# diaoenmao/Multimodal-Controller-for-Generative-Models

Measured on AMD Instinct MI355X. Metric: images/sec (train step) MCGAN CIFAR-10 32x32, higher is better.
Workload: dtype bf16

## Files before the change

multimodal-controller-for-generative-models_amd/csrc/conv_fused.hip:

```cpp
#include "conv_tile.h"
#include <stdlib.h>
#include <type_traits>

namespace {

template <typename T, int BM, int BN, int WM, int WN>
struct ConvCfg {
    static constexpr int NT = 64 * WM * WN;
    static constexpr int FM = BM / WM / 16;
    static constexpr int FN = BN / WN / 16;
    static constexpr int ESZ = Elem<T>::BYTES;
    static constexpr int APITCH = MCGEN_CK * ESZ + 16 * ESZ;
    static constexpr int BROW = MCGEN_CK * ESZ;
    static constexpr int BBYTES = BN * BROW;
    static constexpr int EP = BN + 4;
    static constexpr int NI = (BM * 9 + NT - 1) / NT;
    static constexpr int UPR = BROW / 16;
    static constexpr int UNITS = BN * UPR;
    static constexpr int NU = (UNITS + NT - 1) / NT;
    static constexpr int EPX = (BN >= 128 && BM > 64) ? BM / 64 : 1;
    static constexpr int PPX = BM / EPX;
    static constexpr int CH = BN / 8;
    static constexpr int PROWS = NT / CH;
    static_assert(NT % CH == 0, "epilogue thread mapping");
// ... 1611 lines not shown
    const int H = p.H, N = p.N;
    int tile_m = blockIdx.x;
    int wset = 0;
    if (p.order || p.wsel) {
        const int tpi = (H * W) / BM, pos = tile_m / tpi;
        if (p.wsel) wset = p.wsel[pos];
        if (p.order) tile_m = p.order[pos] * tpi + (tile_m - pos * tpi);
    }
    const int cout0 = blockIdx.y * BN;
    const Geo g = make_geo(BM, tile_m, H, W);
    const int n_img = g.n0 < N ? g.n0 : N - 1;

    f32x4 acc[FN][FM];
#pragma unroll
    for (int i = 0; i < FN; ++i)
#pragma unroll
        for (int j = 0; j < FM; ++j) acc[i][j] = f32x4{0.f, 0.f, 0.f, 0.f};

    const mcgen_seg_t sg0 = seg_for_tile(p.seg[0], g);
    const int C0 = sg0.C;
    const char* wimg = reinterpret_cast<const char*>(p.w) + (size_t)wset * (size_t)p.wsel_stride * 2;
    const size_t wblock_bytes = (size_t)p.Cout_w * BROW;
    auto seg_info = [&](int si, const int16_t*& cidx, int& cw, int& cnt) {
        const mcgen_seg_t& sg = p.seg[si];
        cw = sg.Cw > 0 ? sg.Cw : sg.C;
        cidx = nullptr; cnt = sg.C;
        if (sg.cmap) {
            const int16_t* rec = sg.cmap + (size_t)n_img * sg.cmap_stride;
            cidx = rec + cw;
            cnt = (int)mc_sload(rec + 2 * cw + 32 + 2 * ((cw + 31) >> 5));
            if (cnt > sg.C) cnt = sg.C;
        }
    };
    const int16_t* cidx0 = nullptr; int cw0 = C0, cnt0 = C0;
    if constexpr (GK) seg_info(0, cidx0, cw0, cnt0);
    const int nchunk = GK ? ((cnt0 + 31) >> 5) : (C0 >> 5), T0 = nchunk * 9;
    const size_t tapstride0 = (size_t)(cw0 + 1) * p.Cout_w * 2;

    constexpr int UPR = C::UPR, RPP = 64 / UPR;
    int d_src[PPW];
    int k0_[PPW];
    const int rsub = lane / LPR, ci = lane % LPR;
#pragma unroll
    for (int k = 0; k < PPW; ++k) {
        const int piece = wave * PPW + k;
        if constexpr (!GK) {
            const int row = piece * RPP + lane / UPR, pu = lane % UPR;
            const int lgrp = pu ^ (3 * ((row >> 3) & 1));
            d_src[k] = (cout0 + row < p.Cout_w) ? (cout0 + row) * BROW + lgrp * 16 : (lane % UPR) * 16;
            k0_[k] = 0;
        } else {
            const int rho0 = RPPK * piece, rho = rho0 + rsub;
            k0_[k] = (rho0 < 16) ? 8 * (rho0 >> 2) + (rho0 & 3) : 8 * ((rho0 - 16) >> 2) + 4 + ((rho0 - 16) & 3);
            int co = cout0 + 16 * ((ci >> 1) ^ (rho & 7)) + 8 * (ci & 1);
            if (co > p.Cout_w - 8) co = p.Cout_w - 8;
            d_src[k] = co * 2;
        }
    }
    auto ksel_map = [&](const int16_t* cidx, int t, int k) -> int {
        const uint32_t d01 = mc_sload(cidx + 32 * t + k0_[k]);
        uint32_t sel = d01;
        if constexpr (RPPK == 4) {
            const uint32_t d23 = mc_sload(cidx + 32 * t + k0_[k] + 2);
            sel = (rsub & 2) ? d23 : d01;
        }
        return (int)((rsub & 1) ? (sel >> 16) : (sel & 0xffffu));
    };
    auto ksel = [&](const int16_t* cidx, int cw, int t, int k) -> int {
        if (cidx) return ksel_map(cidx, t, k);
// ... 164 lines not shown
                    for (int i = 0; i < HF; ++i) M::run(wf[fn], af[cs][i], acc[fn][i]);
            } else {
                const int sn = (slot_c + 1 == R) ? 0 : slot_c + 1;
                const char* ldsB = ldsB0 + sn * BB;
#pragma unroll
                for (int fn = 0; fn < FN; ++fn) {
#pragma unroll
                    for (int i = 0; i < HF; ++i) M::run(wf[fn], af[cs][i], acc[fn][HF + i]);
                    wf[fn] = wfrag(ldsB, fn);
                }
            }
            if constexpr (h == 0) {
                asm volatile("s_waitcnt lgkmcnt(0)" ::: "memory");
                pp_wait_vm<pp_vmcnt_b(ph, R, NIW, PPW)>();
                pp_barrier();
            } else {
                slot_c = (slot_c + 1 == R) ? 0 : slot_c + 1;
                ++tcur;
            }
        });
        if constexpr (GK) {
#pragma unroll
            for (int kk = 0; kk < PPW; ++kk) krow_c[kk] = krow_n[kk];
        }
    }
    asm volatile("s_waitcnt vmcnt(0)" ::: "memory");
    }

    if (p.nseg > 1) {
        int tg = 0;
        int nrest = 0;
        const int16_t* cidx1 = nullptr; int cw1 = 8, cnt1 = 0;
        if constexpr (GK) { seg_info(1, cidx1, cw1, cnt1); nrest = (cnt1 + 31) >> 5; }
        else for (int s = 1; s < p.nseg; ++s) nrest += (p.seg[s].C + MCGEN_CK - 1) / MCGEN_CK;
        const char* wseg1 = wimg + 9 * tapstride0;
        const size_t tapstride1 = (size_t)(cw1 + 1) * p.Cout_w * 2;
        auto tail_dma = [&](int t, int slot) {
#pragma unroll
            for (int k = 0; k < PPW; ++k) {
                if constexpr (GK) dma_piece_gk(wseg1, tapstride1, ksel(cidx1, cw1, t, k) * p.Cout_w * 2 + d_src[k], 0, slot, k);
                else dma_piece(T0 + t, slot, k);
            }
        };
        pp_barrier();
        constexpr int SUBW = BM * APITCH;
        constexpr int A2 = 2 * (((PP * APITCH + 1023) / 1024) * 1024);
        constexpr int TGMAX = (A2 + 2 * BB) / SUBW;
#ifndef MCGEN_PP_TG
#define MCGEN_PP_TG 4
#endif
        constexpr int TG = TGMAX < MCGEN_PP_TG ? TGMAX : MCGEN_PP_TG;
        constexpr int NI1 = (BM * 4 + NT - 1) / NT;
        static_assert(TG >= 1 && R >= 5, "tail groups: windows over the window buffers + two ring slots, weights in slots 2 .. 4");
        auto tslot = [](int t) { return 2 + t % 3; };
        auto tail_dma_c = [&](int t) { tail_dma(t < nrest ? t : nrest - 1, tslot(t)); };
        if (nrest > 0) { tail_dma_c(0); tail_dma_c(1); }
        for (int s = 1; s < p.nseg; ++s) {
            const mcgen_seg_t sg = seg_for_tile(p.seg[s], g);
            PatchStager<T, NT, NI1, APITCH> stager;
            stager.setup(sg, g, N, H, W, tid);
            const int b_lane = (wm * (BM / WM) + l15) * APITCH + lg * 16;
            const int nch = GK ? nrest : (sg.C + MCGEN_CK - 1) / MCGEN_CK;
#pragma unroll 1
            for (int q0 = 0; q0 < nch; q0 += TG) {
                const int ng = (nch - q0) < TG ? (nch - q0) : TG;
                if (q0 > 0) __builtin_amdgcn_s_barrier();
                {
                    typename PatchStager<T, NT, NI1, APITCH>::raw_t raw[TG];
#pragma unroll
                    for (int i = 0; i < TG; ++i) if (i < ng) stager.load(sg, (q0 + i) * MCGEN_CK, raw[i]);
#pragma unroll
                    for (int i = 0; i < TG; ++i) if (i < ng) stager.write(sg, (q0 + i) * MCGEN_CK, raw[i], ldsA0 + i * SUBW, g.n0 < N ? g.n0 : -1);
                }
#pragma unroll 1
                for (int i = 0; i < ng; ++i) {
                    if constexpr (PPW == 2) asm volatile("s_waitcnt vmcnt(2)" ::: "memory"); else asm volatile("s_waitcnt vmcnt(1)" ::: "memory");
                    asm volatile("s_waitcnt lgkmcnt(0)" ::: "memory");
                    pp_barrier();
                    tail_dma_c(tg + 2);
                    const char* ldsB = ldsB0 + tslot(tg) * BB;
                    const char* ldsW = ldsA0 + i * SUBW + b_lane;
                    typename M::frag xf[FM], yf[FN];
#pragma unroll
                    for (int fm = 0; fm < FM; ++fm) xf[fm] = *reinterpret_cast<const typename M::frag*>(ldsW + fm * 16 * APITCH);
#pragma unroll
                    for (int fn = 0; fn < FN; ++fn) yf[fn] = wfrag(ldsB, fn);
#pragma unroll
                    for (int fn = 0; fn < FN; ++fn)
#pragma unroll
                        for (int fm = 0; fm < FM; ++fm) M::run(yf[fn], xf[fm], acc[fn][fm]);
                    ++tg;
                }
            }
        }
    }
// ... 256 lines not shown
    auto kern = conv_gk_kernel<BM, BN, WM, WN>;
    static int raised = 0;
    if (int rc = raise_lds(reinterpret_cast<const void*>(kern), lds, &raised)) return rc;
    hipLaunchKernelGGL(kern, dim3(mt, nt), dim3(C::NT), lds, st, *p, a_bytes);
    MCGEN_LAUNCH_CHECK("conv_fused(gk)");
    return 0;
}

static int dispatch_gk(const mcgen_conv_t* p, int dtype, hipStream_t st) {
    MCGEN_CHECK(dtype == MCGEN_BF16, "conv_fused: K-major launches are bf16");
    for (int s = 0; s < p->nseg; ++s) {
        const mcgen_seg_t& g = p->seg[s];
        const int cw = g.Cw > 0 ? g.Cw : g.C;
        MCGEN_CHECK(cw % 8 == 0 && cw <= 2048 && g.C <= cw + 32, "conv_fused(gk): segment %d: bad channel counts C=%d Cw=%d", s, g.C, cw);
        MCGEN_CHECK(g.cmap || g.C == cw, "conv_fused(gk): segment %d: compacted channels need the map that orders them", s);
        MCGEN_CHECK(!g.cmap || g.cmap_stride >= 2 * cw + 32, "conv_fused(gk): segment %d: map stride too small", s);
        MCGEN_CHECK(!g.cmap || g.code == nullptr, "conv_fused(gk): segment %d: the code of a compacted segment rides in its scale / shift rows", s);
    }
    MCGEN_CHECK(p->Cout_w % 8 == 0 && p->Cout_w >= 64, "conv_fused(gk): at least 64 output channels");
    int bm = 0, bn = 0;
    MCGEN_CHECK(mc_tile(p, &bm, &bn), "conv_fused(gk): no tile of a %dx%d map lies inside one image", p->H, p->W);
    static const long pp_mode = env_long("MCGEN_PP", 7);
    if (bm == 256 && bn == 256 && (pp_mode & 4) && pp_fits_<256, 256, 2, 4, 5, true>(p)) return launch_pp<bf16_t, 256, 256, 2, 4, 5, true>(p, st);
    if (bm == 256 && bn == 256) return launch_gk<256, 256, 2, 4>(p, st);
    if (bm == 128 && bn == 256) return launch_gk<128, 256, 2, 4>(p, st);
    return launch_gk<128, 128, 2, 2>(p, st);
}

template <int BM, int BN, int WM, int WN, int R, bool GK>
static bool pp_fits_(const mcgen_conv_t* p) {
    using C = ConvCfg<bf16_t, BM, BN, WM, WN>;
    if (p->w_layout != (GK ? 2 : 0) || p->H * p->W < BM || (p->W != 16 && p->W != 32)) return false;
    if (p->seg[0].ksize != 3 || p->seg[0].C % MCGEN_CK != 0 || p->seg[0].C < 2 * MCGEN_CK || p->seg[0].C > C::NT) return false;
    if ((p->seg[0].cmap != nullptr) != GK) return false;
    for (int s = 1; s < p->nseg; ++s) if (p->seg[s].ksize != 1 || (!GK && p->seg[s].cmap)) return false;
    const int PP = mcgen_patch_pixels(BM, p->H, p->W, 3);
    if (PP * 4 > PP_NIW_MAX * C::NT || PP * 4 <= C::NT) return false;
    const int a_bytes = round_up(PP * C::APITCH, 1024);
    const int lds = 2 * a_bytes + R * C::BBYTES + p->seg[0].C * 8 + 16;
    return lds <= 160 * 1024;
}
template <int BM, int BN, int WM, int WN, int R>
static bool pp_fits(const mcgen_conv_t* p) { return pp_fits_<BM, BN, WM, WN, R, false>(p); }
template <typename T, int BM, int BN, int WM, int WN, int R, bool GK>
static int launch_pp(const mcgen_conv_t* p, hipStream_t st) {
    static_assert(sizeof(T) == 2, "the pp form is bf16");
    using C = ConvCfg<bf16_t, BM, BN, WM, WN>;
    const long Mtot = (long)p->N * p->H * p->W;
    const int mt = (int)(Mtot / BM);
    const int nt = (p->Cout_w + BN - 1) / BN;
    const int PP = mcgen_patch_pixels(BM, p->H, p->W, 3);
    const int a_bytes = round_up(PP * C::APITCH, 1024);
    int lds = 2 * a_bytes + R * C::BBYTES + p->seg[0].C * 8 + 16;
    const int epi_bytes = C::PPX * C::EP * 4 + (p->ycmap ? YTAB_BYTES : 0), red_bytes = C::PROWS * BN * 2 * 4;
    const int epi_fast = (BM / PP_EPI_PASSES(BM, BN)) * C::EP * 4 + (p->ycmap ? YTAB_BYTES : 0);
    if (epi_bytes > lds) lds = epi_bytes;
    if (epi_fast > lds) lds = epi_fast;
    if (red_bytes > lds) lds = red_bytes;
    MCGEN_CHECK(lds <= 160 * 1024, "conv_fused(pp): tile %dx%d needs %d bytes of LDS", BM, BN, lds);
    void (*kern)(const mcgen_conv_t, const int) = p->W == 32 ? conv_pp_kernel<BM, BN, WM, WN, R, 5, GK> : conv_pp_kernel<BM, BN, WM, WN, R, 4, GK>;
#ifdef MCGEN_TUNING
    static const long abl = env_long("MCGEN_PP_ABL", 0);
    if (abl == 2 && p->W == 32) kern = conv_pp_kernel<BM, BN, WM, WN, R, 5, GK, 2>;
#endif
#ifdef MCGEN_TUNING
    int raised_now = 0;
    if (int rc = raise_lds(reinterpret_cast<const void*>(kern), lds, &raised_now)) return rc;
#else
// ... 41 lines not shown
#endif
    };
    *n = (int)(sizeof(t) / sizeof(t[0]));
    return t;
}

static int dispatch(const mcgen_conv_t* p, int dtype, const TilePick& t, hipStream_t st) {
    int n = 0;
    const CfgEntry* tab = dtype == MCGEN_BF16 ? bf16_table(&n) : f32_table(&n);
    for (int i = 0; i < n; ++i)
        if (tab[i].BM == t.BM && tab[i].BN == t.BN && tab[i].pipe == t.pipe) return tab[i].fn(p, st);
    return mcgen_fail("conv_fused: no instantiation for tile %dx%d pipe=%d dtype=%d", t.BM, t.BN, t.pipe, dtype);
}

static int validate(const mcgen_conv_t* p) {
    MCGEN_CHECK(p && p->nseg >= 1 && p->nseg <= 2, "conv_fused: nseg must be 1 or 2");
    MCGEN_CHECK(p->N > 0 && ilog2_exact(p->H) >= 0 && ilog2_exact(p->W) >= 0, "conv_fused: H and W must be powers of two (got %dx%d)", p->H, p->W);
    MCGEN_CHECK(p->W <= 64 && p->H * p->W >= 1, "conv_fused: W up to 64 supported");
    MCGEN_CHECK(p->Cout > 0 && p->Cout_w == round_up(p->Cout, 16), "conv_fused: Cout_w must be Cout rounded up to 16");
    MCGEN_CHECK(p->Cy % 8 == 0 && p->Cy > 0, "conv_fused: Cy must be a positive multiple of 8");
    MCGEN_CHECK(p->w && p->y, "conv_fused: null weight image or output");
    for (int s = 0; s < p->nseg; ++s) {
        const mcgen_seg_t& g = p->seg[s];
        MCGEN_CHECK(g.x && g.C > 0 && g.C % 8 == 0, "conv_fused: segment %d: C must be a positive multiple of 8", s);
        MCGEN_CHECK(g.ksize == 1 || g.ksize == 3, "conv_fused: segment %d: ksize must be 1 or 3", s);
        MCGEN_CHECK(!g.ups || (p->H >= 2 && p->W >= 2), "conv_fused: upsampled segment needs H, W >= 2");
        MCGEN_CHECK(g.group_n >= 0 && (g.group_n == 0 || p->N % g.group_n == 0), "conv_fused: segment %d: group_n must divide N", s);
    }
    if (p->pool) MCGEN_CHECK(p->H >= 2 && p->W >= 2, "conv_fused: pooling needs H, W >= 2");
    MCGEN_CHECK(p->stats_mode >= 0 && p->stats_mode <= 2, "conv_fused: bad stats_mode");
    MCGEN_CHECK(p->stats_mode != 2 || (p->gate_x && p->gmean && p->grstd), "conv_fused: stats_mode 2 needs gate_x, gmean, grstd");
    MCGEN_CHECK(p->stats_mode == 0 || p->stats, "conv_fused: stats_mode set without a stats buffer");
    MCGEN_CHECK(p->w_layout >= 0 && p->w_layout <= 2, "conv_fused: unknown weight layout %d", p->w_layout);
    if (p->wsel || p->order) {
        MCGEN_CHECK(p->w_layout == 0 && (p->y_group == 0 || !p->order), "conv_fused: per-mode weight sets (wsel / order) go with the chunked weight image (w_layout 0)");
        MCGEN_CHECK(!p->wsel || p->wsel_stride > 0, "conv_fused: wsel needs wsel_stride");
    }
    if (p->yperm) {
        MCGEN_CHECK(p->wsel && !p->order && !p->ycmap, "conv_fused: permuted weight rows (yperm) come with wsel, without order / ycmap");
        MCGEN_CHECK(!p->pool && !p->res && !p->gate_x && !p->ocode && !p->tanh_out, "conv_fused: a compacted output takes bias and statistics only");
        MCGEN_CHECK(p->Cy % 8 == 0 && p->Cy <= p->Cout && p->Cout % 8 == 0 && p->Cout_w == p->Cout && p->Cout_w <= 256 && p->yperm_stride >= p->Cout && p->yperm_stride % 8 == 0,
                    "conv_fused: yperm: bad pitch %d / stride %d for %d channels", p->Cy, p->yperm_stride, p->Cout);
    }
    if (p->ycmap) {
        MCGEN_CHECK(!p->pool && !p->res && !p->gate_x && !p->ocode && !p->tanh_out && !p->bias2, "conv_fused: a compacted output takes bias and statistics only");
        MCGEN_CHECK(p->Cy % 32 == 0 && p->Cy <= round_up(p->Cout, 8) + 32 && p->ycmap_stride >= 2 * round_up(p->Cout, 8) + 32,
                    "conv_fused: compacted output: bad pitch %d / map stride %d", p->Cy, p->ycmap_stride);
        MCGEN_CHECK(p->Cout_w <= 256, "conv_fused: a compacted output needs all channels in one tile");
    } else if (!p->yperm) {
        MCGEN_CHECK(p->Cy >= p->Cout, "conv_fused: Cy must be >= Cout");
    }
    return 0;
}

}

extern "C" int mcgen_conv_m_tiles(const mcgen_conv_t* p, int dtype) {
    if (!p) return 0;
    if (p->w_layout != 0) {
        int bm = 0, bn = 0;
        if (!mc_tile(p, &bm, &bn)) return 0;
        return (int)(((long)p->N * p->H * p->W + bm - 1) / bm);
    }
    if (mcgen_conv_smap_ok(p, dtype)) return p->N;
    if (const int bm = mcgen_conv_px1_bm(p, dtype)) return (int)((long)p->N * p->H * p->W / bm);
    const TilePick t = pick_tile(p, dtype);
// ... 2 lines not shown
}

extern "C" int mcgen_conv_tile(const mcgen_conv_t* p, int dtype, int* bm, int* bn) {
    if (!p || !bm || !bn) return mcgen_fail("conv_tile: null pointer");
    if (p->w_layout != 0) {
        MCGEN_CHECK(mc_tile(p, bm, bn), "conv_tile: no K-major tile for a %dx%d map", p->H, p->W);
        return 0;
    }
    const TilePick t = pick_tile(p, dtype);
    *bm = t.BM; *bn = t.BN;
    return 0;
}

extern "C" int mcgen_conv_form(const mcgen_conv_t* p, int dtype) {
    if (!p || p->w_layout != 0 || p->order) return 0;
    if (p->wsel) return mcgen_conv_head_ok(p, dtype) ? 5 : 0;
    if (mcgen_conv_skinny_ok(p, dtype)) return 1;
    if (mcgen_conv_smap_ok(p, dtype)) return 2;
    if (mcgen_conv_px1_bm(p, dtype)) return 3;
    if (mcgen_conv_c8_ok(p, dtype)) return 4;
    if (mcgen_conv_head_ok(p, dtype)) return 5;
    return 0;
}

extern "C" int mcgen_conv_fused(const mcgen_conv_t* p, int dtype, void* stream) {
    if (int rc = validate(p)) return rc;
    if (p->y_group != 0) {
        MCGEN_CHECK(mcgen_conv_head_ok(p, dtype), "conv_fused: the paired output layout (y_group) is built for the image head only "
                    "(bf16, one 3x3 segment to <= 8 channels of pitch 8 on 32x32 maps, N %% y_group == 0)");
        return mcgen_conv_head(p, reinterpret_cast<hipStream_t>(stream));
    }
    if (p->w_layout == 1) return dispatch_mc(p, dtype, reinterpret_cast<hipStream_t>(stream));
    if (p->w_layout == 2) return dispatch_gk(p, dtype, reinterpret_cast<hipStream_t>(stream));
    for (int s = 0; s < p->nseg; ++s) MCGEN_CHECK(p->seg[s].cmap == nullptr, "conv_fused: a compaction map needs a K-major launch (w_layout 1 or 2)");
    if (p->wsel && mcgen_conv_head_ok(p, dtype)) return mcgen_conv_head(p, reinterpret_cast<hipStream_t>(stream));
    if (p->wsel || p->order) {
        const TilePick tw = pick_tile(p, dtype);
        MCGEN_CHECK(dtype == MCGEN_BF16 && tw.pipe == 20, "conv_fused: per-mode weight sets need the software-pipelined bf16 form "
                    "(3x3 first segment of 64 .. 512 channels in whole chunks, 16x16 / 32x32 maps, >= 65536 pixels)");
        if (p->ycmap) MCGEN_CHECK(tw.BM <= p->H * p->W && p->Cout_w <= tw.BN, "conv_fused: compacted output: the %dx%d tile must hold all %d channels", tw.BM, tw.BN, p->Cout_w);
        if (p->yperm) MCGEN_CHECK(tw.BM <= p->H * p->W && p->Cout_w == tw.BN, "conv_fused: yperm: the %dx%d tile must hold exactly the %d channels", tw.BM, tw.BN, p->Cout_w);
        return dispatch(p, dtype, tw, reinterpret_cast<hipStream_t>(stream));
    }
    if (mcgen_conv_skinny_ok(p, dtype)) return mcgen_conv_skinny(p, reinterpret_cast<hipStream_t>(stream));
    if (mcgen_conv_smap_ok(p, dtype)) return mcgen_conv_smap(p, reinterpret_cast<hipStream_t>(stream));
    if (mcgen_conv_px1_bm(p, dtype)) return mcgen_conv_px1(p, reinterpret_cast<hipStream_t>(stream));
    if (mcgen_conv_c8_ok(p, dtype)) return mcgen_conv_c8(p, reinterpret_cast<hipStream_t>(stream));
    if (mcgen_conv_head_ok(p, dtype)) return mcgen_conv_head(p, reinterpret_cast<hipStream_t>(stream));
    const TilePick t = pick_tile(p, dtype);
    if (p->ycmap) MCGEN_CHECK(dtype == MCGEN_BF16 && t.BM <= p->H * p->W && p->Cout_w <= t.BN,
                              "conv_fused: compacted output: the %dx%d tile must lie inside one image and hold all %d channels", t.BM, t.BN, p->Cout_w);
    MCGEN_CHECK(t.BM >= 2 * p->W || p->H * p->W <= t.BM, "conv_fused: tile of %d pixels too small for W=%d", t.BM, p->W);
    for (int s = 0; s < p->nseg; ++s) {
        const int ti = t.BM > p->H * p->W ? t.BM / (p->H * p->W) : 1;
        MCGEN_CHECK(p->seg[s].group_n == 0 || p->seg[s].group_n % ti == 0,
                    "conv_fused: a tile of %d images would straddle BatchNorm groups of %d images", ti, p->seg[s].group_n);
    }
    hipStream_t st = reinterpret_cast<hipStream_t>(stream);
    if (dtype != MCGEN_F32 && dtype != MCGEN_BF16) return mcgen_fail("conv_fused: unknown dtype %d", dtype);
    return dispatch(p, dtype, t, st);
}
#endif
```

multimodal-controller-for-generative-models_amd/csrc/conv_head.hip:

```cpp
#include "conv_tile.h"

namespace {

constexpr int HD_NT = 512, HD_W = 32, HD_ROWS = 8;
constexpr int HD_PC = HD_W + 2, HD_PP = (HD_ROWS + 2) * HD_PC;
constexpr int HD_PITCH = 80;
constexpr int HD_BUF = ((HD_PP * HD_PITCH + 127) / 128) * 128;
constexpr int HD_NI = (HD_PP * 4 + HD_NT - 1) / HD_NT;

__global__ __launch_bounds__(HD_NT, 4)
void conv_head_kernel(const mcgen_conv_t p) {
    extern __shared__ __attribute__((aligned(16))) char smem[];
    const int tid = threadIdx.x, lane = tid & 63;
    const int wv = __builtin_amdgcn_readfirstlane(tid >> 6);
    const int l15 = lane & 15, lg = lane >> 4;
    const int n = blockIdx.x >> 2, h0 = (blockIdx.x & 3) * HD_ROWS;
    const mcgen_seg_t sg = p.seg[0];
    const int C = sg.C, nchunk = C >> 5;
    const float* anyf = reinterpret_cast<const float*>(p.w);
    const size_t arow = sg.group_n > 0 ? (size_t)(n / sg.group_n) * C : 0;
    const float* scp = sg.scale ? sg.scale + arow : anyf;
    const float* shp = sg.scale ? sg.shift + arow : anyf;
    const float* cdp = sg.code ? sg.code + (size_t)n * C : anyf;
    const float relu_lo = sg.relu ? 0.f : -__builtin_inff();

    const int u = tid & 3;
    int src[HD_NI], dst[HD_NI];
#pragma unroll
    for (int k = 0; k < HD_NI; ++k) {
        const int wp = (tid >> 2) + 128 * k;
        const int wr = wp / HD_PC, wc = wp - wr * HD_PC;
        const int h = h0 + wr - 1, w = wc - 1;
        dst[k] = wp < HD_PP ? wp * HD_PITCH + u * 16 : -1;
        src[k] = (wp < HD_PP && (unsigned)h < (unsigned)HD_W && (unsigned)w < (unsigned)HD_W) ? ((n * HD_W + h) * HD_W + w) * C + u * 8 : -1;
    }
    const bf16_t* xs = reinterpret_cast<const bf16_t*>(sg.x);
    u32x4 raw[HD_NI];
    float sc[8], sh[8], cd[8];
    auto load_chunk = [&](int q) {
#pragma unroll
        for (int k = 0; k < HD_NI; ++k) raw[k] = *reinterpret_cast<const u32x4*>(xs + (src[k] >= 0 ? (size_t)src[k] + q * 32 : 0));
        load8f(sg.scale ? scp + q * 32 + u * 8 : anyf, sc);
        load8f(sg.scale ? shp + q * 32 + u * 8 : anyf, sh);
        load8f(sg.code ? cdp + q * 32 + u * 8 : anyf, cd);
    };
    auto write_chunk = [&](char* buf) {
#pragma unroll
        for (int k = 0; k < HD_NI; ++k) {
            if (dst[k] < 0) continue;
            union { bf16x8 h; u32x4 w; } o;
#pragma unroll
// ... 29 lines not shown
            }
        }
        if (q + 1 < nchunk) write_chunk(smem + ((q + 1) & 1) * HD_BUF);
    }
    if (lg < 2) {
        float bs[4];
#pragma unroll
        for (int r = 0; r < 4; ++r) {
            const int co = 4 * lg + r;
            bs[r] = (p.bias && co < p.Cout) ? p.bias[co] : 0.f;
            if (p.bias2 && co < p.Cout) bs[r] += p.bias2[co];
        }
        const int ny = p.y_group > 0 ? (n / p.y_group) * 2 * p.y_group + p.y_group + n % p.y_group : n;
        bf16_t* y = reinterpret_cast<bf16_t*>(p.y) + ((size_t)(ny * HD_W + h0 + wv) * HD_W) * p.Cy + 4 * lg;
#pragma unroll
        for (int f = 0; f < 2; ++f) {
            union { bf16_t h[4]; uint2 w; } o;
#pragma unroll
            for (int r = 0; r < 4; ++r) {
                float v = fmaf(acc[f][r], p.alpha, bs[r]);
                if (p.tanh_out) v = tanhf(v);
                o.h[r] = (bf16_t)((4 * lg + r) < p.Cout ? v : 0.f);
            }
            *reinterpret_cast<uint2*>(y + (size_t)(16 * f + l15) * p.Cy) = o.w;
        }
    }
}

}

int mcgen_conv_head_ok(const mcgen_conv_t* p, int dtype) {
    if (dtype != MCGEN_BF16 || p->w_layout != 0 || p->nseg != 1) return 0;
    const mcgen_seg_t& g = p->seg[0];
    if (g.ksize != 3 || g.ups || g.cmap || g.C % 32 || g.C < 64 || g.group_n < 0 || (g.group_n > 0 && p->N % g.group_n)) return 0;
    if (p->H != HD_W || p->W != HD_W || p->Cout > 8 || p->Cout_w != 16 || p->Cy != 8) return 0;
    if (p->pool || p->res || p->ocode || p->gate_x || p->stats_mode || p->ycmap || p->order) return 0;
    if ((long)p->N * HD_W * HD_W * g.C >= (1L << 31)) return 0;
    if (p->y_group < 0 || (p->y_group > 0 && p->N % p->y_group)) return 0;
    return 1;
}

int mcgen_conv_head(const mcgen_conv_t* p, hipStream_t st) {
    static bool raised = false;
    if (!raised) {
        raised = true;
        hipError_t e = hipFuncSetAttribute(reinterpret_cast<const void*>(conv_head_kernel), hipFuncAttributeMaxDynamicSharedMemorySize, 2 * HD_BUF);
        if (e != hipSuccess) return mcgen_fail("conv_head: cannot raise LDS limit: %s", hipGetErrorString(e));
    }
    hipLaunchKernelGGL(conv_head_kernel, dim3(p->N * 4), dim3(HD_NT), 2 * HD_BUF, st, *p);
    MCGEN_LAUNCH_CHECK("conv_head");
    return 0;
}
```

multimodal-controller-for-generative-models_amd/gan_engine.py:

```python
from __future__ import annotations

from typing import Dict, List, Optional

import torch
import torch.nn as nn

from . import ops
from ._tuning import flag as _flag
from .ops import Seg

Tensor = torch.Tensor


def _bump(t: Tensor):
    torch.autograd.graph.increment_version(t)


class FlatState:

    def __init__(self, tensors: List[Tensor]):
        self.tensors = tensors
        self.flat: Optional[Tensor] = None
        self.offsets: List[int] = []
        self._index = {id(t): i for i, t in enumerate(tensors)}
# ... 378 lines not shown
        c0 = lin.out_features // 16
        x0, st = ops.conv_fused([Seg(zt, ksize=1)], self.img['lin'], 16 * c0, bias=self.img['lin_bias'],
                                stats_mode=st_mode)
        x = x0.view(n, 4, 4, c0)
        fold = 16
        ctx['zt'] = zt
        blocks_ctx = []
        codes = self._codes.run_any(indicator)
        gk = groups > 1 and one_hot and self._gk_enabled()
        hint = getattr(indicator, '_mcgen_onehot', None)
        pm = gk and self._pm_enabled() and hint is not None and hint[0].shape[0] * hint[1] == n
        wsel = None
        if pm:
            wsel = hint[2] if len(hint) > 2 and hint[2] is not None else hint[0].to(torch.int32).repeat(hint[1])
        x_cm = None
        cmaps = self._gather_cmaps(self._pm_need(), wsel) if pm else {}
        caps_h = [self._cap(b.mc_2) if (gk and self._gk_block(i)) else None for i, b in enumerate(res)]
        for i, b in enumerate(res):
            s = x.shape[1]
            code1, code2 = codes[2 * i], codes[2 * i + 1]
            bn1 = _bn_forward(b.conv[0].module, st, ng * s * s, train, fold, groups)
            fold = 1
            co = b.conv[4].module.out_channels
            ci = b.conv[4].module.in_channels
            cap_h = caps_h[i]
            nxt = res[i + 1] if i + 1 < len(res) else None
            ymc = self._y_mc(i, pm and 'headm' in self.img) if cap_h is not None else None
            cap_y = self._cap(ymc) if ymc is not None else None
            cm_h = (cmaps[id(b.mc_2)] if id(b.mc_2) in cmaps else ops.mc_cmap(code2)) if cap_h else None
            cm_y = (cmaps[id(ymc)] if id(ymc) in cmaps else ops.mc_cmap(codes[2 * (i + 1)])) if cap_y else None
            if x_cm is not None:
                sa, ta = ops.mc_affine(code1, x_cm[0], x_cm[1], bn1.scale, bn1.shift, group_n=gn)
                if pm and f'b{i}.w1m' in self.img:
                    seg_a = Seg(x, scale=sa, shift=ta, ups=True, relu=True, group_n=1)
                    h, st_h = ops.conv_fused([seg_a], self.img[f'b{i}.w1m'], co, bias=b.conv[4].module.bias, stats_mode=st_mode,
                                             cy=cap_h, wsel=wsel, yperm=self._mode_perms(b.mc_2))
                else:
                    seg_a = Seg(x, scale=sa, shift=ta, ups=True, relu=True, group_n=1, cmap=x_cm[0], cw=ci)
                    h, st_h = ops.conv_fused([seg_a], self.img[f'b{i}.w1g'], co, bias=b.conv[4].module.bias, stats_mode=st_mode,
                                             kmajor=2, ycmap=cm_h, cy=cap_h)
            else:
                mc = self._mc_block(i) and f'b{i}.w1k' in self.img
                cm1 = ops.mc_cmap(code1) if mc else None
                seg_a = Seg(x, scale=bn1.scale, shift=bn1.shift, code=code1, ups=True, relu=True, group_n=gn, cmap=cm1)
                h, st_h = ops.conv_fused([seg_a], self.img[f'b{i}.w1k' if mc else f'b{i}.w1'], co, bias=b.conv[4].module.bias,
                                         stats_mode=st_mode, kmajor=int(mc), ycmap=cm_h, cy=cap_h)
            bn2 = _bn_forward(b.conv[5].module, st_h, ng * 4 * s * s, train, 1, groups)
            if cm_h is not None:
                sb, tb = ops.mc_affine(code2, cm_h, cap_h, bn2.scale, bn2.shift, group_n=gn)
                use_pm = pm and f'b{i}.w2sm' in self.img
                seg_b = Seg(h, scale=sb, shift=tb, relu=True, group_n=1) if use_pm else \
                    Seg(h, scale=sb, shift=tb, relu=True, group_n=1, cmap=cm_h, cw=co)
                if x_cm is not None:
                    ss, ts = ops.mc_affine(code1, x_cm[0], x_cm[1])
                    seg_s = Seg(x, ksize=1, scale=ss, shift=ts, ups=True, group_n=1) if use_pm else \
                        Seg(x, ksize=1, scale=ss, shift=ts, ups=True, group_n=1, cmap=x_cm[0], cw=ci)
                else:
                    seg_s = Seg(x, ksize=1, code=code1, ups=True)
                if use_pm:
                    y, st = ops.conv_fused([seg_b, seg_s], self.img[f'b{i}.w2sm'].view(-1), co, bias=b.conv[8].module.bias,
                                           bias2=b.shortcut[2].module.bias, stats_mode=st_mode, cy=cap_y, wsel=wsel,
                                           yperm=self._mode_perms(ymc) if ymc is not None else None)
                else:
                    y, st = ops.conv_fused([seg_b, seg_s], self.img[f'b{i}.w2sk'], co,
                                           bias=b.conv[8].module.bias.detach() + b.shortcut[2].module.bias.detach(),
                                           stats_mode=st_mode, kmajor=2, ycmap=cm_y, cy=cap_y)
            else:
                seg_b = Seg(h, scale=bn2.scale, shift=bn2.shift, code=code2, relu=True, group_n=gn)
                seg_s = Seg(x, ksize=1, code=code1, ups=True)
                y, st = ops.conv_fused([seg_b, seg_s], self.img[f'b{i}.w2s'], co, bias=b.conv[8].module.bias,
                                       bias2=b.shortcut[2].module.bias, stats_mode=st_mode)
            blocks_ctx.append(dict(x=x, h=h, code1=code1, code2=code2, bn1=bn1, bn2=bn2))
            x = y
            x_cm = (cm_y, cap_y) if cm_y is not None else None
        s = x.shape[1]
        bnh = _bn_forward(head_bn, st, ng * s * s, train, fold, groups)
        codeh = codes[-1]
        hw, hsel = self.img['head'], None
        if x_cm is not None:
            sh_, th_ = ops.mc_affine(codeh, x_cm[0], x_cm[1], bnh.scale, bnh.shift, group_n=gn)
            seg_h = Seg(x, scale=sh_, shift=th_, relu=True, group_n=1)
            hw, hsel = self.img['headm'], wsel
        else:
            seg_h = Seg(x, scale=bnh.scale, shift=bnh.shift, code=codeh, relu=True, group_n=gn)
        cimg = head_conv.out_channels
        if pair_out is not None:
            if tuple(pair_out.shape) != (2 * n, x.shape[1], x.shape[2], ops.pad8(cimg)) or pair_out.dtype != dt:
                raise McgenError(f'pair_out must be {(2 * n, x.shape[1], x.shape[2], ops.pad8(cimg))} {dt}')
            direct = (dt == torch.bfloat16 and x.shape[1] == 32 and x.shape[2] == 32 and cimg <= 8 and x.shape[-1] % 32 == 0
                      and x.shape[-1] >= 64 and n * 32 * 32 * x.shape[-1] < (1 << 31))
            if direct:
                ops.conv_fused([seg_h], hw, cimg, bias=head_conv.bias, tanh=True, out=pair_out, y_group=ng, wsel=hsel)
                out = None
            else:
                out, _ = ops.conv_fused([seg_h], hw, cimg, bias=head_conv.bias, tanh=True, wsel=hsel)
                pv = pair_out.view(groups, 2 * ng, *pair_out.shape[1:])
                pv[:, ng:].copy_(out.view(groups, ng, *out.shape[1:]))
        else:
            out, _ = ops.conv_fused([seg_h], hw, cimg, bias=head_conv.bias, tanh=True, wsel=hsel)
        ctx.update(blocks=blocks_ctx, y=x, bnh=bnh, codeh=codeh, out=out)
        _flush_counters()
        if pair_out is not None:
            return None, ctx
        return (Nhwc(out, head_conv.out_channels) if nhwc else ops.to_nchw(out, head_conv.out_channels)), ctx

    def backward(self, ctx, dimg: Tensor, gflat: Tensor, accumulate: bool = False):
        for _ in self.backward_iter(ctx, dimg, gflat, accumulate, split=False):
            pass

    def bucket_cut(self) -> int:
        lin, res, head_bn, head_mc, head_conv = self._layers()
        return max(1, len(res) // 2) if len(res) > 1 else 0

    def backward_iter(self, ctx, dimg: Tensor, gflat: Tensor, accumulate: bool = False, split: bool = True):
# ... 506 lines not shown
```

multimodal-controller-for-generative-models_amd/ops.py:

```python
from __future__ import annotations

import ctypes as C
import os as _os
from dataclasses import dataclass
from typing import Optional, Sequence, Tuple

import torch

from . import _lib
from ._lib import check
from ._tuning import flag as _flag

Tensor = torch.Tensor


def _dt(dtype: torch.dtype) -> int:
    if dtype == torch.float32:
        return _lib.F32
    if dtype == torch.bfloat16:
        return _lib.BF16
    raise _lib.McgenError(f'unsupported compute dtype {dtype}')


def _stream() -> int:
# ... 97 lines not shown
           'event_pair_overhead_us': over_ms * 1e3, 'flops_per_launch': flops / cnt,
           'algorithmic_bytes_per_launch': nbytes / cnt, 'split_k_bytes_per_launch': extra / cnt,
           'intensity_flop_per_byte': intensity, 'machine_balance_flop_per_byte': balance,
           'by_kernel': {k: {'launches': v[0] / np_, 'total_ms': v[1] * 1e3 / np_, 'tflops': v[2] / v[1] / 1e12,
                             'gbytes_per_s': v[4] / v[1] / 1e9, **({'split_k_gbytes_per_s': v[5] / v[1] / 1e9} if v[5] else {})}
                         for k, v in sorted(agg.items(), key=lambda kv: -kv[1][1])}}
    if hbm:
        out.update(achieved=nbytes / secs / 1e9, peak=HBM_PEAK_BYTES_PER_S / 1e9, unit='GB/s',
                   frac=nbytes / secs / HBM_PEAK_BYTES_PER_S)
    return out


def pad8(c: int) -> int:
    return (c + 7) // 8 * 8


def pad16(c: int) -> int:
    return (c + 15) // 16 * 16


@dataclass
class Seg:
    x: Tensor
    ksize: int = 3
    scale: Optional[Tensor] = None
    shift: Optional[Tensor] = None
    code: Optional[Tensor] = None
    ups: bool = False
    relu: bool = False
    group_n: int = 0
    cmap: Optional[Tensor] = None
    cw: int = 0

    def fill(self, s: _lib.Seg):
        s.x = _p(self.x)
        s.scale, s.shift, s.code = _f32(self.scale), _f32(self.shift), _f32(self.code)
        s.C = self.x.shape[-1]
        s.ups, s.relu, s.ksize = int(self.ups), int(self.relu), self.ksize
        s.group_n = int(self.group_n)
        s.cmap, s.cmap_stride, s.Cw = None, 0, int(self.cw)
        if self.cmap is not None:
            cm = self.cw or s.C
            if self.cmap.dtype != torch.int16 or tuple(self.cmap.shape) != (self.x.shape[0], cmap_stride(cm)):
                raise _lib.McgenError(f'cmap must be int16 {(self.x.shape[0], cmap_stride(cm))}, got {self.cmap.dtype} {tuple(self.cmap.shape)}')
            s.cmap, s.cmap_stride = _p(self.cmap), self.cmap.shape[1]
        if self.group_n and self.scale is not None:
            g = self.x.shape[0] // self.group_n
            if self.x.shape[0] % self.group_n or tuple(self.scale.shape) != (g, s.C) or tuple(self.shift.shape) != (g, s.C):
                raise _lib.McgenError(f'grouped BatchNorm affine must be {(g, s.C)}, got {tuple(self.scale.shape)}')
        if self.code is not None and tuple(self.code.shape) != (self.x.shape[0], self.x.shape[-1]):
            raise _lib.McgenError(f'code shape {tuple(self.code.shape)} does not match x {tuple(self.x.shape)}')


def to_nhwc(x: Tensor, dtype: torch.dtype, cp: Optional[int] = None, out: Optional[Tensor] = None) -> Tensor:
    n, c, h, w = x.shape
    cp = cp or pad8(c)
    y = out if out is not None else torch.empty((n, h, w, cp), dtype=dtype, device=x.device)
    if tuple(y.shape) != (n, h, w, cp) or y.dtype != dtype or not y.is_contiguous():
        raise _lib.McgenError(f'to_nhwc: out must be a contiguous {(n, h, w, cp)} {dtype} tensor')
    check(_lib.load().mcgen_nchw_to_nhwc(_f32(x.contiguous()), _p(y), _dt(dtype), n, c, h, w, cp, _stream()), 'nchw_to_nhwc')
    return y


def to_nchw(x: Tensor, c: int) -> Tensor:
    n, h, w, cp = x.shape
    y = torch.empty((n, c, h, w), dtype=torch.float32, device=x.device)
    check(_lib.load().mcgen_nhwc_to_nchw(_p(x), _f32(y), _dt(x.dtype), n, c, h, w, cp, _stream()), 'nhwc_to_nchw')
    return y


def pool2_sum(x: Tensor) -> Tensor:
    n, h, w, c = x.shape
    y = torch.empty((n, h // 2, w // 2, c), dtype=x.dtype, device=x.device)
    check(_lib.load().mcgen_pool2_sum(_p(x), _p(y), _dt(x.dtype), n, h // 2, w // 2, c, _stream()), 'pool2_sum')
    return y


# ... 90 lines not shown
    n = weight_image_elems(cout, cin, ks, transpose)
    if out is None:
        out = torch.empty(n, dtype=dtype, device=w.device)
    assert out.numel() == n and out.dtype == dtype
    check(_lib.load().mcgen_prep_weight(_f32(w), _p(out), _dt(dtype), cout, cin, ks, int(transpose), row_perm,
                                        _f32(sigma), float(wscale), _stream()), 'prep_weight')
    return out


def conv_fused(segs: Sequence[Seg], wimg: Tensor, cout: int, *, bias: Optional[Tensor] = None, bias2: Optional[Tensor] = None,
               pool: bool = False, alpha: float = 1.0, res: Optional[Tensor] = None,
               ocode: Optional[Tensor] = None, gate_x: Optional[Tensor] = None,
               gscale: Optional[Tensor] = None, gshift: Optional[Tensor] = None,
               gmean: Optional[Tensor] = None, grstd: Optional[Tensor] = None,
               tanh: bool = False, stats_mode: int = 0, cy: Optional[int] = None,
               out: Optional[Tensor] = None, kmajor: int = 0, ycmap: Optional[Tensor] = None,
               y_group: int = 0, wsel: Optional[Tensor] = None, order: Optional[Tensor] = None,
               yperm: Optional[Tensor] = None) -> Tuple[Tensor, Optional[Tensor]]:
    s0 = segs[0]
    n = s0.x.shape[0]
    h = s0.x.shape[1] * (2 if s0.ups else 1)
    w = s0.x.shape[2] * (2 if s0.ups else 1)
    dtype = s0.x.dtype
    cy = cy or pad8(cout)
    ho, wo = (h // 2, w // 2) if pool else (h, w)
    p = _lib.Conv()
    p.nseg = len(segs)
    for i, s in enumerate(segs):
        if s.x.dtype != dtype:
            raise _lib.McgenError('all segments must share the compute dtype')
        hs = s.x.shape[1] * (2 if s.ups else 1)
        if hs != h or s.x.shape[0] != n:
            raise _lib.McgenError('segments disagree on the convolution resolution')
        s.fill(p.seg[i])
    if wimg.dtype != dtype:
        raise _lib.McgenError(f'weight image dtype {wimg.dtype} != activation dtype {dtype}')
    if kmajor:
        need = sum(s.ksize * s.ksize * ((s.cw or s.x.shape[-1]) + 1) for s in segs) * pad16(cout)
    else:
        need = sum(((s.x.shape[-1] + 31) // 32) * s.ksize * s.ksize for s in segs) * pad16(cout) * 32
    if wsel is not None:
        if wsel.dtype != torch.int32 or wsel.numel() != n or (order is not None and (order.dtype != torch.int32 or order.numel() != n)):
            raise _lib.McgenError('wsel / order must be int32 [N]')
        if wimg.numel() % need:
            raise _lib.McgenError(f'weight sets: {wimg.numel()} elements are not a multiple of one image ({need})')
    elif order is not None:
        raise _lib.McgenError('order comes with wsel')
    elif wimg.numel() != need:
        raise _lib.McgenError(f'weight image has {wimg.numel()} elements, the segments need {need}')
    y = out if out is not None else torch.empty((n, ho, wo, cy), dtype=dtype, device=s0.x.device)
    if y_group:
        if out is None or tuple(y.shape) != (2 * n, ho, wo, cy) or y.dtype != dtype or not y.is_contiguous():
            raise _lib.McgenError(f'y_group: `out` must be a contiguous {(2 * n, ho, wo, cy)} {dtype} buffer')
    else:
        assert tuple(y.shape) == (n, ho, wo, cy) and y.dtype == dtype
    p.w, p.bias, p.y = _p(wimg), _f32(bias), _p(y)
    p.bias2 = _f32(bias2)
    p.N, p.H, p.W = n, h, w
    p.Cout, p.Cout_w, p.Cy = cout, pad16(cout), cy
    p.pool, p.alpha = int(pool), float(alpha)
    for name, t in (('res', res), ('gate_x', gate_x)):
        if t is not None and (tuple(t.shape) != (n, ho, wo, cy) or t.dtype != dtype):
            raise _lib.McgenError(f'{name} must be {(n, ho, wo, cy)} {dtype}, got {tuple(t.shape)} {t.dtype}')
    if ocode is not None and tuple(ocode.shape) != (n, cout):
        raise _lib.McgenError(f'ocode must be {(n, cout)}')
    p.res, p.ocode, p.gate_x = _p(res), _f32(ocode), _p(gate_x)
    p.gscale, p.gshift, p.gmean, p.grstd = _f32(gscale), _f32(gshift), _f32(gmean), _f32(grstd)
    p.tanh_out, p.stats_mode = int(tanh), stats_mode
    p.w_layout = int(kmajor)
    p.y_group = int(y_group)
    p.wsel, p.wsel_stride, p.order = _p(wsel), (need if wsel is not None else 0), _p(order)
    p.yperm, p.yperm_stride = None, 0
    if yperm is not None:
        if wsel is None or yperm.dtype != torch.int16 or yperm.dim() != 2 or yperm.shape[0] * need != wimg.numel() or not yperm.is_contiguous():
            raise _lib.McgenError('yperm must be a contiguous int16 [sets, stride] table that comes with wsel')
        p.yperm, p.yperm_stride = _p(yperm), yperm.shape[1]
    p.ycmap, p.ycmap_stride = None, 0
    if ycmap is not None:
        if ycmap.dtype != torch.int16 or tuple(ycmap.shape) != (n, cmap_stride(pad8(cout))):
            raise _lib.McgenError(f'ycmap must be int16 {(n, cmap_stride(pad8(cout)))}')
        p.ycmap, p.ycmap_stride = _p(ycmap), ycmap.shape[1]
    stats = None
# ... 1249 lines not shown
```

Measured before the change: 18090.

## Skip inactive channel chunks in per-mode weight-set convolutions via mode compaction maps

```diff
diff --git a/multimodal-controller-for-generative-models_amd/csrc/conv_fused.hip b/multimodal-controller-for-generative-models_amd/csrc/conv_fused.hip
--- a/multimodal-controller-for-generative-models_amd/csrc/conv_fused.hip
+++ b/multimodal-controller-for-generative-models_amd/csrc/conv_fused.hip
@@ -1667,9 +1667,18 @@
             if (cnt > sg.C) cnt = sg.C;
         }
     };
+    auto seg_chunks = [&](int si) -> int {
+        const mcgen_seg_t& sg = p.seg[si];
+        const int all = (sg.C + MCGEN_CK - 1) / MCGEN_CK;
+        if (GK || !p.wsel || !sg.cmap) return all;
+        const int16_t* rec = sg.cmap + (size_t)wset * sg.cmap_stride;
+        const int kc = ((int)mc_sload(rec + 2 * sg.Cw + 32 + 2 * ((sg.Cw + 31) >> 5)) + MCGEN_CK - 1) / MCGEN_CK;
+        return kc < all ? kc : all;
+    };
     const int16_t* cidx0 = nullptr; int cw0 = C0, cnt0 = C0;
     if constexpr (GK) seg_info(0, cidx0, cw0, cnt0);
-    const int nchunk = GK ? ((cnt0 + 31) >> 5) : (C0 >> 5), T0 = nchunk * 9;
+    const int nchunk = GK ? ((cnt0 + 31) >> 5) : seg_chunks(0), T0 = nchunk * 9;
+    const int T1 = (C0 >> 5) * 9;
     const size_t tapstride0 = (size_t)(cw0 + 1) * p.Cout_w * 2;
 
     constexpr int UPR = C::UPR, RPP = 64 / UPR;
@@ -1900,14 +1909,14 @@
         int nrest = 0;
         const int16_t* cidx1 = nullptr; int cw1 = 8, cnt1 = 0;
         if constexpr (GK) { seg_info(1, cidx1, cw1, cnt1); nrest = (cnt1 + 31) >> 5; }
-        else for (int s = 1; s < p.nseg; ++s) nrest += (p.seg[s].C + MCGEN_CK - 1) / MCGEN_CK;
+        else for (int s = 1; s < p.nseg; ++s) nrest += seg_chunks(s);
         const char* wseg1 = wimg + 9 * tapstride0;
         const size_t tapstride1 = (size_t)(cw1 + 1) * p.Cout_w * 2;
         auto tail_dma = [&](int t, int slot) {
 #pragma unroll
             for (int k = 0; k < PPW; ++k) {
                 if constexpr (GK) dma_piece_gk(wseg1, tapstride1, ksel(cidx1, cw1, t, k) * p.Cout_w * 2 + d_src[k], 0, slot, k);
-                else dma_piece(T0 + t, slot, k);
+                else dma_piece(T1 + t, slot, k);
             }
         };
         pp_barrier();
@@ -1928,7 +1937,7 @@
             PatchStager<T, NT, NI1, APITCH> stager;
             stager.setup(sg, g, N, H, W, tid);
             const int b_lane = (wm * (BM / WM) + l15) * APITCH + lg * 16;
-            const int nch = GK ? nrest : (sg.C + MCGEN_CK - 1) / MCGEN_CK;
+            const int nch = GK ? nrest : seg_chunks(s);
 #pragma unroll 1
             for (int q0 = 0; q0 < nch; q0 += TG) {
                 const int ng = (nch - q0) < TG ? (nch - q0) : TG;
@@ -2251,8 +2260,8 @@
     using C = ConvCfg<bf16_t, BM, BN, WM, WN>;
     if (p->w_layout != (GK ? 2 : 0) || p->H * p->W < BM || (p->W != 16 && p->W != 32)) return false;
     if (p->seg[0].ksize != 3 || p->seg[0].C % MCGEN_CK != 0 || p->seg[0].C < 2 * MCGEN_CK || p->seg[0].C > C::NT) return false;
-    if ((p->seg[0].cmap != nullptr) != GK) return false;
-    for (int s = 1; s < p->nseg; ++s) if (p->seg[s].ksize != 1 || (!GK && p->seg[s].cmap)) return false;
+    if (GK ? p->seg[0].cmap == nullptr : (p->seg[0].cmap && !p->wsel)) return false;
+    for (int s = 1; s < p->nseg; ++s) if (p->seg[s].ksize != 1 || (!GK && p->seg[s].cmap && !p->wsel)) return false;
     const int PP = mcgen_patch_pixels(BM, p->H, p->W, 3);
     if (PP * 4 > PP_NIW_MAX * C::NT || PP * 4 <= C::NT) return false;
     const int a_bytes = round_up(PP * C::APITCH, 1024);
@@ -2360,6 +2369,13 @@
     MCGEN_CHECK(p->stats_mode != 2 || (p->gate_x && p->gmean && p->grstd), "conv_fused: stats_mode 2 needs gate_x, gmean, grstd");
     MCGEN_CHECK(p->stats_mode == 0 || p->stats, "conv_fused: stats_mode set without a stats buffer");
     MCGEN_CHECK(p->w_layout >= 0 && p->w_layout <= 2, "conv_fused: unknown weight layout %d", p->w_layout);
+    for (int s = 0; s < p->nseg && p->w_layout == 0; ++s) {
+        const mcgen_seg_t& g = p->seg[s];
+        if (!g.cmap) continue;
+        MCGEN_CHECK(p->wsel, "conv_fused: a compaction map needs a K-major launch (w_layout 1 or 2) or per-mode weight sets (wsel)");
+        MCGEN_CHECK(g.Cw >= g.C && g.cmap_stride >= mcgen_cmap_stride(g.Cw), "conv_fused: segment %d: the sets' compaction records "
+                    "need Cw = their channels (>= C) and a stride of at least mcgen_cmap_stride(Cw)", s);
+    }
     if (p->wsel || p->order) {
         MCGEN_CHECK(p->w_layout == 0 && (p->y_group == 0 || !p->order), "conv_fused: per-mode weight sets (wsel / order) go with the chunked weight image (w_layout 0)");
         MCGEN_CHECK(!p->wsel || p->wsel_stride > 0, "conv_fused: wsel needs wsel_stride");
@@ -2428,7 +2444,6 @@
     }
     if (p->w_layout == 1) return dispatch_mc(p, dtype, reinterpret_cast<hipStream_t>(stream));
     if (p->w_layout == 2) return dispatch_gk(p, dtype, reinterpret_cast<hipStream_t>(stream));
-    for (int s = 0; s < p->nseg; ++s) MCGEN_CHECK(p->seg[s].cmap == nullptr, "conv_fused: a compaction map needs a K-major launch (w_layout 1 or 2)");
     if (p->wsel && mcgen_conv_head_ok(p, dtype)) return mcgen_conv_head(p, reinterpret_cast<hipStream_t>(stream));
     if (p->wsel || p->order) {
         const TilePick tw = pick_tile(p, dtype);
diff --git a/multimodal-controller-for-generative-models_amd/csrc/conv_head.hip b/multimodal-controller-for-generative-models_amd/csrc/conv_head.hip
--- a/multimodal-controller-for-generative-models_amd/csrc/conv_head.hip
+++ b/multimodal-controller-for-generative-models_amd/csrc/conv_head.hip
@@ -16,7 +16,13 @@
     const int l15 = lane & 15, lg = lane >> 4;
     const int n = blockIdx.x >> 2, h0 = (blockIdx.x & 3) * HD_ROWS;
     const mcgen_seg_t sg = p.seg[0];
-    const int C = sg.C, nchunk = C >> 5;
+    const int C = sg.C;
+    int nchunk = C >> 5;
+    if (p.wsel && sg.cmap) {
+        const int16_t* rec = sg.cmap + (size_t)p.wsel[n] * sg.cmap_stride;
+        const int kc = (*reinterpret_cast<const int32_t*>(rec + 2 * sg.Cw + 32 + 2 * ((sg.Cw + 31) >> 5)) + 31) >> 5;
+        if (kc < nchunk) nchunk = kc;
+    }
     const float* anyf = reinterpret_cast<const float*>(p.w);
     const size_t arow = sg.group_n > 0 ? (size_t)(n / sg.group_n) * C : 0;
     const float* scp = sg.scale ? sg.scale + arow : anyf;
@@ -112,7 +118,7 @@
 int mcgen_conv_head_ok(const mcgen_conv_t* p, int dtype) {
     if (dtype != MCGEN_BF16 || p->w_layout != 0 || p->nseg != 1) return 0;
     const mcgen_seg_t& g = p->seg[0];
-    if (g.ksize != 3 || g.ups || g.cmap || g.C % 32 || g.C < 64 || g.group_n < 0 || (g.group_n > 0 && p->N % g.group_n)) return 0;
+    if (g.ksize != 3 || g.ups || (g.cmap && !p->wsel) || g.C % 32 || g.C < 64 || g.group_n < 0 || (g.group_n > 0 && p->N % g.group_n)) return 0;
     if (p->H != HD_W || p->W != HD_W || p->Cout > 8 || p->Cout_w != 16 || p->Cy != 8) return 0;
     if (p->pool || p->res || p->ocode || p->gate_x || p->stats_mode || p->ycmap || p->order) return 0;
     if ((long)p->N * HD_W * HD_W * g.C >= (1L << 31)) return 0;
diff --git a/multimodal-controller-for-generative-models_amd/gan_engine.py b/multimodal-controller-for-generative-models_amd/gan_engine.py
--- a/multimodal-controller-for-generative-models_amd/gan_engine.py
+++ b/multimodal-controller-for-generative-models_amd/gan_engine.py
@@ -434,7 +434,7 @@
             if x_cm is not None:
                 sa, ta = ops.mc_affine(code1, x_cm[0], x_cm[1], bn1.scale, bn1.shift, group_n=gn)
                 if pm and f'b{i}.w1m' in self.img:
-                    seg_a = Seg(x, scale=sa, shift=ta, ups=True, relu=True, group_n=1)
+                    seg_a = Seg(x, scale=sa, shift=ta, ups=True, relu=True, group_n=1, cmap=self._mode_maps(b.mc_1), cw=ci)
                     h, st_h = ops.conv_fused([seg_a], self.img[f'b{i}.w1m'], co, bias=b.conv[4].module.bias, stats_mode=st_mode,
                                              cy=cap_h, wsel=wsel, yperm=self._mode_perms(b.mc_2))
                 else:
@@ -451,11 +451,11 @@
             if cm_h is not None:
                 sb, tb = ops.mc_affine(code2, cm_h, cap_h, bn2.scale, bn2.shift, group_n=gn)
                 use_pm = pm and f'b{i}.w2sm' in self.img
-                seg_b = Seg(h, scale=sb, shift=tb, relu=True, group_n=1) if use_pm else \
+                seg_b = Seg(h, scale=sb, shift=tb, relu=True, group_n=1, cmap=self._mode_maps(b.mc_2), cw=co) if use_pm else \
                     Seg(h, scale=sb, shift=tb, relu=True, group_n=1, cmap=cm_h, cw=co)
                 if x_cm is not None:
                     ss, ts = ops.mc_affine(code1, x_cm[0], x_cm[1])
-                    seg_s = Seg(x, ksize=1, scale=ss, shift=ts, ups=True, group_n=1) if use_pm else \
+                    seg_s = Seg(x, ksize=1, scale=ss, shift=ts, ups=True, group_n=1, cmap=self._mode_maps(b.mc_1), cw=ci) if use_pm else \
                         Seg(x, ksize=1, scale=ss, shift=ts, ups=True, group_n=1, cmap=x_cm[0], cw=ci)
                 else:
                     seg_s = Seg(x, ksize=1, code=code1, ups=True)
@@ -481,7 +481,7 @@
         hw, hsel = self.img['head'], None
         if x_cm is not None:
             sh_, th_ = ops.mc_affine(codeh, x_cm[0], x_cm[1], bnh.scale, bnh.shift, group_n=gn)
-            seg_h = Seg(x, scale=sh_, shift=th_, relu=True, group_n=1)
+            seg_h = Seg(x, scale=sh_, shift=th_, relu=True, group_n=1, cmap=self._mode_maps(head_mc), cw=head_conv.in_channels)
             hw, hsel = self.img['headm'], wsel
         else:
             seg_h = Seg(x, scale=bnh.scale, shift=bnh.shift, code=codeh, relu=True, group_n=gn)
diff --git a/multimodal-controller-for-generative-models_amd/ops.py b/multimodal-controller-for-generative-models_amd/ops.py
--- a/multimodal-controller-for-generative-models_amd/ops.py
+++ b/multimodal-controller-for-generative-models_amd/ops.py
@@ -153,7 +153,7 @@
     cmap: Optional[Tensor] = None
     cw: int = 0
 
-    def fill(self, s: _lib.Seg):
+    def fill(self, s: _lib.Seg, sets: int = 0):
         s.x = _p(self.x)
         s.scale, s.shift, s.code = _f32(self.scale), _f32(self.shift), _f32(self.code)
         s.C = self.x.shape[-1]
@@ -162,8 +162,9 @@
         s.cmap, s.cmap_stride, s.Cw = None, 0, int(self.cw)
         if self.cmap is not None:
             cm = self.cw or s.C
-            if self.cmap.dtype != torch.int16 or tuple(self.cmap.shape) != (self.x.shape[0], cmap_stride(cm)):
-                raise _lib.McgenError(f'cmap must be int16 {(self.x.shape[0], cmap_stride(cm))}, got {self.cmap.dtype} {tuple(self.cmap.shape)}')
+            rows = sets or self.x.shape[0]
+            if self.cmap.dtype != torch.int16 or tuple(self.cmap.shape) != (rows, cmap_stride(cm)):
+                raise _lib.McgenError(f'cmap must be int16 {(rows, cmap_stride(cm))}, got {self.cmap.dtype} {tuple(self.cmap.shape)}')
             s.cmap, s.cmap_stride = _p(self.cmap), self.cmap.shape[1]
         if self.group_n and self.scale is not None:
             g = self.x.shape[0] // self.group_n
@@ -320,7 +321,6 @@
         hs = s.x.shape[1] * (2 if s.ups else 1)
         if hs != h or s.x.shape[0] != n:
             raise _lib.McgenError('segments disagree on the convolution resolution')
-        s.fill(p.seg[i])
     if wimg.dtype != dtype:
         raise _lib.McgenError(f'weight image dtype {wimg.dtype} != activation dtype {dtype}')
     if kmajor:
@@ -336,6 +336,8 @@
         raise _lib.McgenError('order comes with wsel')
     elif wimg.numel() != need:
         raise _lib.McgenError(f'weight image has {wimg.numel()} elements, the segments need {need}')
+    for i, s in enumerate(segs):
+        s.fill(p.seg[i], sets=wimg.numel() // need if (wsel is not None and not kmajor) else 0)
     y = out if out is not None else torch.empty((n, ho, wo, cy), dtype=dtype, device=s0.x.device)
     if y_group:
         if out is None or tuple(y.shape) != (2 * n, ho, wo, cy) or y.dtype != dtype or not y.is_contiguous():
```

Measured after the change: 18290, median of 6. +1.1%, better.
